# Developer-Zer0/GIF-synthesis-with-Discrete-Diffusion

Hardware: NVIDIA B200
Metric: reverse_step_token_updates_per_sec (higher is better)
Workload: dtype f32

## Files before the change

### gif-synthesis-with-discrete-diffusion_b200/csrc/d3pm_step_rows.cuh

```cuda
#pragma once

#include "d3pm_common.cuh"

namespace d3pm {

struct StepParams {
  const float* logits_c;
  const float* logits_u;
  const int64_t* x_t;
  const int64_t* t;
  const float* coef_table;
  const float* gumbel;
  int64_t* x_prev;
  float* post;
  float* recon;
  float* gap;
  uint32_t* status;
  int32_t B, N, K, T;
  int64_t pitch_logits, pitch_gumbel, pitch_out;
  float guidance_scale;
  int32_t sample_mode;
  int32_t gumbel_is_uniform;
  uint64_t seed, offset;
  int64_t row_offset;
  float thin_factor;
  int64_t rows;
  int32_t sample_from;
  float* score;
  const float* sharpen;
  float* winner_post;
  int32_t logits_dtype;
  PhiloxRoundKeys keys;
};

__device__ __forceinline__ float to_log2_units(float m) { return __fmul_rn(m, kLog2e); }

__device__ __forceinline__ float ln_rel_sum(float M, float S) {
  const float m2 = to_log2_units(M);
  const float delta = -fmaf(M, kLog2e, -m2);
  return kLn2 * (lg2(S) + delta);
}

struct RowMath {
  float A, Bc;
  float Pj;
  float PK;
  float Ptot;
  uint32_t j;

  __device__ __forceinline__ void init(const RowCoef& cf, bool masked, float pj, uint32_t jj, int K) {
    init(cf, masked, pj, 1.0f - pj, jj, K);
  }
  __device__ __forceinline__ void init(const RowCoef& cf, bool masked, float pj, float qj, uint32_t jj, int K) {
    j = jj;
    const float eL = masked ? cf.W + kTiny : fmaf(cf.W, qj, fmaf(cf.WS, pj, kTiny));
    A = cf.A;
    Bc = cf.BO * eL;
    Pj = masked ? 0.0f : fmaf(pj, cf.AS, cf.BOS * eL);
    PK = fmaf(cf.PK1, eL, cf.PK0);
    Ptot = masked ? fmaf(static_cast<float>(K), Bc, A) + PK
                  : fmaf(static_cast<float>(K - 1), Bc, A * qj) + Pj + PK;
  }
  __device__ __forceinline__ void init_recon(float pj, uint32_t jj) {
    j = jj;
    A = 1.0f, Bc = 0.0f, Pj = pj, PK = kPFloor, Ptot = 1.0f + kPFloor;
  }
  __device__ __forceinline__ float post_of(uint32_t k, float e, float r) const {
    const float p = fminf(fmaxf(e * r, kPFloor), 1.0f);
    const float P = (k == j) ? Pj : fmaf(p, A, Bc);
    return log_prob_clamped(P);
  }
  __device__ __forceinline__ float post_self() const { return log_prob_clamped(Pj); }
  __device__ __forceinline__ float post_mask() const { return log_prob_clamped(PK); }
};

constexpr float kDefaultThin = 8.0f;
struct ThinRule {
  float scaleA, thrB, accept;
  __device__ __forceinline__ ThinRule(const RowMath& rm, float thin_factor) {
    const float c = thin_factor > 0.f ? thin_factor : kDefaultThin;
    const float inv = __fdividef(c, rm.Ptot);
    scaleA = rm.A * inv * 0.0078125f;
    thrB = fmaf(rm.Bc * inv, 0.0078125f, 1.0f) + 2.384185791015625e-7f;
    accept = -lg2(inv) * kLn2 + 0.02f;
  }
};

constexpr int kRowThreads = 256;

template <int NV, int NW, typename Sync>
__device__ __forceinline__ void group_max_sum_n(float (&m)[NV], float (&s)[NV], float* scratch, Sync sync) {
  const int lane = threadIdx.x & 31, warp = (threadIdx.x >> 5) % NW;
#pragma unroll
  for (int v = 0; v < NV; ++v) {
    const float mw = warp_max(m[v]);
    const float sw =
        warp_sum(m[v] == -CUDART_INF_F ? 0.0f : s[v] * ex2(to_log2_units(m[v]) - to_log2_units(mw)));
    if (lane == 0) {
      scratch[(2 * v) * NW + warp] = mw;
      scratch[(2 * v + 1) * NW + warp] = sw;
    }
  }
  sync();
#pragma unroll
  for (int v = 0; v < NV; ++v) {
    float M = scratch[(2 * v) * NW];
#pragma unroll
    for (int w = 1; w < NW; ++w) M = fmaxf(M, scratch[(2 * v) * NW + w]);
    const float M2 = to_log2_units(M);
    float S = 0.0f;
#pragma unroll
    for (int w = 0; w < NW; ++w) {
      const float mwv = scratch[(2 * v) * NW + w];
      S += (mwv == -CUDART_INF_F) ? 0.0f : scratch[(2 * v + 1) * NW + w] * ex2(to_log2_units(mwv) - M2);
    }
    m[v] = M;
    s[v] = S;
  }
}

template <int V, bool HAS_U, bool THIN>
__global__ void __launch_bounds__(kRowThreads) step_rows_kernel(const StepParams p) {
  constexpr int NW = kRowThreads / 32;
  __shared__ float sred[3][4 * NW];
  __shared__ unsigned long long skey[2][NW];
  __shared__ float sgap[NW];
  const CtaSync sync;

  const int tid = threadIdx.x;
  const int64_t row = blockIdx.x;
  const int b = static_cast<int>(row / p.N);
  const int K = p.K, nq = K >> 2;

  long long tt = p.t[b];
  long long jj = p.x_t[row];
  uint32_t st = 0;
  if (tt < 0 || tt >= p.T) {
    st |= D3PM_STATUS_BAD_T;
    tt = tt < 0 ? 0 : p.T - 1;
  }
  if (jj < 0 || jj > K) {
    st |= D3PM_STATUS_BAD_TOKEN;
    jj = K;
  }
  if (st != 0 && tid == 0 && p.status != nullptr) atomicOr(p.status, st);
  const bool masked = (jj == K);
  const uint32_t j = static_cast<uint32_t>(jj);
  const RowCoef cf = load_row_coef(p.coef_table, static_cast<int>(tt), masked);

  const float* __restrict__ rc = p.logits_c + row * p.pitch_logits;
  const float* __restrict__ ru = HAS_U ? p.logits_u + row * p.pitch_logits : nullptr;

  float x[V][4], z[V][4];
  int nvalid = 0;
#pragma unroll
  for (int i = 0; i < V; ++i) {
    const int q = tid + i * kRowThreads;
    if (q < nq) {
      nvalid = i + 1;
      const float4 a = ld_stream4(rc + 4 * q);
      x[i][0] = a.x, x[i][1] = a.y, x[i][2] = a.z, x[i][3] = a.w;
      if (HAS_U) {
        const float4 c = ld_stream4(ru + 4 * q);
        z[i][0] = c.x, z[i][1] = c.y, z[i][2] = c.z, z[i][3] = c.w;
      }
    } else {
#pragma unroll
      for (int e = 0; e < 4; ++e) x[i][e] = -CUDART_INF_F, z[i][e] = -CUDART_INF_F;
    }
  }
  float xj = 0.f, zj = 0.f;
  if (!masked) {
    xj = __ldg(rc + j);
    if (HAS_U) zj = __ldg(ru + j);
  }

  float m[2] = {-CUDART_INF_F, -CUDART_INF_F}, s[2] = {0.f, 0.f};
#pragma unroll
  for (int i = 0; i < V; ++i)
#pragma unroll
    for (int e = 0; e < 4; ++e) {
      m[0] = fmaxf(m[0], x[i][e]);
      if (HAS_U) m[1] = fmaxf(m[1], z[i][e]);
    }
  {
// ... 260 lines not shown
```

### gif-synthesis-with-discrete-diffusion_b200/csrc/d3pm_step_stream.cuh

```cuda
#pragma once

#include <cuda_fp16.h>

#include <type_traits>

#include "d3pm_step_rows.cuh"

namespace d3pm {

constexpr int kGroupThreads = 128;
constexpr int kGroupWarps = kGroupThreads / 32;
constexpr int kGroupsPerCta = 4;
constexpr int kStreamThreads = kGroupThreads * kGroupsPerCta;
constexpr int kCandPerRow = 30;
constexpr float kStreamThin = 8.0f;
constexpr float kRedoThin = 16.0f;
constexpr int kCoefSmemRows = 256;
struct RowInfo {
  float A, Bc, Pj, PK, accept;
  uint32_t j;
  int32_t rel;
  int32_t pad;
};

template <int NP, int CPT, bool HAS_U>
struct StreamShape {
  static_assert(CPT == 8 || (CPT == 16 && !HAS_U), "64 classes per thread only fit in registers without the second tensor");
  static constexpr int K = 1024 * NP;
  static constexpr int GT = 256 * NP / CPT;
  static constexpr int NW = GT / 32;
  static constexpr int NG = kStreamThreads / GT;
  static constexpr int SB = 128 / NG;
  static constexpr int RC = 8192 / NG;
  static constexpr int PS = 128 / GT;
  static constexpr int NCALL = CPT / 2;
  static_assert(GT >= 32 && GT <= 128 && NG <= 16, "unsupported group shape");
};

template <int NP, int CPT, bool HAS_U>
struct __align__(128) GroupSmem {
  using Sh = StreamShape<NP, CPT, HAS_U>;
  float c[1024 * NP];
  float u[HAS_U ? 1024 * NP : 4];
  alignas(16) float red[3][6 * 4];
  unsigned long long full;
  unsigned long long keys[4];
  uint32_t redo_cnt;
  uint32_t pad;
  RowInfo info[Sh::SB];
  uint32_t cand_cnt[Sh::SB];
  uint32_t cand_k[Sh::SB][kCandPerRow];
  float cand_p[Sh::SB][kCandPerRow];
  int32_t redo[Sh::RC];
};

__device__ __forceinline__ uint32_t smem_u32(const void* p) {
  return static_cast<uint32_t>(__cvta_generic_to_shared(p));
}
__device__ __forceinline__ void mbar_init(unsigned long long* bar, uint32_t count) {
  asm volatile("mbarrier.init.shared::cta.b64 [%0], %1;" ::"r"(smem_u32(bar)), "r"(count) : "memory");
  asm volatile("fence.mbarrier_init.release.cluster;" ::: "memory");
}
__device__ __forceinline__ void mbar_expect_tx(unsigned long long* bar, uint32_t bytes) {
  asm volatile("mbarrier.arrive.expect_tx.shared::cta.b64 _, [%0], %1;" ::"r"(smem_u32(bar)), "r"(bytes) : "memory");
}
__device__ __forceinline__ void mbar_wait(unsigned long long* bar, uint32_t parity) {
  const uint32_t addr = smem_u32(bar);
  uint32_t done;
  do {
    asm volatile(
        "{\n\t.reg .pred p;\n\t"
        "mbarrier.try_wait.parity.shared::cta.b64 p, [%1], %2;\n\t"
        "selp.u32 %0, 1, 0, p;\n\t}"
        : "=r"(done)
        : "r"(addr), "r"(parity)
        : "memory");
  } while (!done);
}
__device__ __forceinline__ void tma_load_row(void* dst, const void* src, uint32_t bytes, unsigned long long* bar) {
  asm volatile(
      "cp.async.bulk.shared::cluster.global.mbarrier::complete_tx::bytes [%0], [%1], %2, [%3];"
      ::"r"(smem_u32(dst)), "l"(src), "r"(bytes), "r"(smem_u32(bar))
      : "memory");
}
__device__ __forceinline__ void group_bar(int id) {
  asm volatile("bar.sync %0, %1;" ::"r"(id), "n"(kGroupThreads) : "memory");
}
struct GroupSync {
  int id;
  __device__ __forceinline__ void operator()() const { group_bar(id); }
};
template <int NW>
struct StreamSync {
  int id;
  __device__ __forceinline__ void operator()() const {
    if (NW == 1) __syncwarp();
    else asm volatile("bar.sync %0, %1;" ::"r"(id), "n"(32 * NW) : "memory");
  }
};
__device__ __forceinline__ float4 lds4(const float* p) { return *reinterpret_cast<const float4*>(p); }
template <int LD>
struct LogitType {
  static constexpr uint32_t kBytes = LD == D3PM_LOGITS_F32 ? 4u : 2u;
  static __device__ __forceinline__ float2 widen(uint32_t pair) {
    if constexpr (LD == D3PM_LOGITS_BF16) {
      return make_float2(__uint_as_float(pair << 16), __uint_as_float(pair & 0xffff0000u));
    } else {
      return __half22float2(*reinterpret_cast<const __half2*>(&pair));
    }
  }
  static __device__ __forceinline__ void chunk(const float* stage, int q, float2& lo, float2& hi) {
    if constexpr (LD == D3PM_LOGITS_F32) {
      const float4 a = lds4(stage + 4 * q);
      lo = make_float2(a.x, a.y), hi = make_float2(a.z, a.w);
    } else {
      const uint2 raw = *reinterpret_cast<const uint2*>(reinterpret_cast<const unsigned char*>(stage) + 8 * q);
      lo = widen(raw.x), hi = widen(raw.y);
    }
  }
  static __device__ __forceinline__ float one(const float* stage, uint32_t k) {
    if constexpr (LD == D3PM_LOGITS_F32) {
      return stage[k];
    } else {
      const uint32_t h = reinterpret_cast<const unsigned short*>(stage)[k];
      if constexpr (LD == D3PM_LOGITS_BF16) return __uint_as_float(h << 16);
      else return __half2float(__ushort_as_half(static_cast<unsigned short>(h)));
    }
  }
  static __device__ __forceinline__ const void* row(const float* base, unsigned long long elements) {
    return reinterpret_cast<const unsigned char*>(base) + elements * kBytes;
  }
};
template <int NW>
__device__ __forceinline__ float4 lds_warps(const float* p, float neutral) {
  if (NW == 4) return lds4(p);
  const float2 a = *reinterpret_cast<const float2*>(p);
  return make_float4(a.x, a.y, neutral, neutral);
}
template <int NW, int NV, typename Sync>
__device__ __forceinline__ void stream_max_sum(float (&m)[NV], float (&s)[NV], float* scratch, Sync sync) {
  const int lane = threadIdx.x & 31, warp = (threadIdx.x >> 5) & (NW - 1);
#pragma unroll
  for (int v = 0; v < NV; ++v) {
    const float mw = warp_max(m[v]);
    const float mw2 = to_log2_units(mw);
    const float sw = warp_sum(s[v] * ex2(to_log2_units(m[v]) - mw2));
    if (NW == 1) {
      m[v] = mw, s[v] = sw;
    } else if (lane == 0) {
      scratch[(3 * v) * 4 + warp] = mw;
      scratch[(3 * v + 1) * 4 + warp] = mw2;
      scratch[(3 * v + 2) * 4 + warp] = sw;
    }
  }
  sync();
  if constexpr (NW > 1) {
#pragma unroll
  for (int v = 0; v < NV; ++v) {
    const float4 mw = lds_warps<NW>(scratch + (3 * v) * 4, -CUDART_INF_F), mw2 = lds_warps<NW>(scratch + (3 * v + 1) * 4, 0.f);
    const float4 sw = lds_warps<NW>(scratch + (3 * v + 2) * 4, 0.f);
    if (NW == 4) {
      const float M = fmaxf(fmaxf(mw.x, mw.y), fmaxf(mw.z, mw.w));
      const float M2 = to_log2_units(M);
      m[v] = M;
      s[v] = fmaf(sw.x, ex2(mw2.x - M2), fmaf(sw.y, ex2(mw2.y - M2), fmaf(sw.z, ex2(mw2.z - M2), sw.w * ex2(mw2.w - M2))));
    } else {
      const float M = fmaxf(mw.x, mw.y);
      const float M2 = to_log2_units(M);
      m[v] = M;
      s[v] = fmaf(sw.x, ex2(mw2.x - M2), sw.y * ex2(mw2.y - M2));
    }
  }
  }
}

__device__ __forceinline__ float warp_min(float x) {
  float m;
  asm volatile("redux.sync.min.f32 %0, %1, 0xffffffff;" : "=f"(m) : "f"(x));
  return m;
}

template <int NW, int NV, typename Sync>
__device__ __forceinline__ void stream_max(float* mx, float* scratch, Sync sync) {
  const int lane = threadIdx.x & 31, warp = (threadIdx.x >> 5) & (NW - 1);
#pragma unroll
  for (int v = 0; v < NV; ++v) {
    const float a = warp_max(mx[v]);
    if (NW == 1) mx[v] = a;
    else if (lane == 0) scratch[v * 4 + warp] = a;
  }
  sync();
  if constexpr (NW > 1) {
#pragma unroll
  for (int v = 0; v < NV; ++v) {
    const float4 a = lds_warps<NW>(scratch + v * 4, -CUDART_INF_F);
    mx[v] = fmaxf(fmaxf(a.x, a.y), fmaxf(a.z, a.w));
  }
  }
}

template <int NW, int NV, typename Sync>
__device__ __forceinline__ void stream_sum(float (&s)[NV], float* scratch, Sync sync) {
  const int lane = threadIdx.x & 31, warp = (threadIdx.x >> 5) & (NW - 1);
#pragma unroll
  for (int v = 0; v < NV; ++v) {
    const float sw = warp_sum(s[v]);
    if (NW == 1) s[v] = sw;
    else if (lane == 0) scratch[v * 4 + warp] = sw;
  }
  sync();
  if constexpr (NW > 1) {
#pragma unroll
  for (int v = 0; v < NV; ++v) {
    const float4 a = lds_warps<NW>(scratch + v * 4, 0.f);
    s[v] = (a.x + a.y) + (a.z + a.w);
  }
  }
}

template <int NW, typename Sync>
__device__ __forceinline__ unsigned long long stream_max_u64(unsigned long long key, unsigned long long* scratch, Sync sync) {
  const int lane = threadIdx.x & 31, warp = (threadIdx.x >> 5) & (NW - 1);
  key = warp_max_u64(key);
  if (NW == 1) {
    sync();
    return key;
  }
  if (lane == 0) scratch[warp] = key;
  sync();
  unsigned long long best = scratch[0];
#pragma unroll
  for (int w = 1; w < NW; ++w) best = scratch[w] > best ? scratch[w] : best;
  return best;
}

template <int NP, int CPT, bool HAS_U>
__device__ __noinline__ void score_batch(GroupSmem<NP, CPT, HAS_U>& S, int nslots, const ParamNoiseStream& rng, const StepParams& p, int G,
                                         int first_row) {
  using Sh = StreamShape<NP, CPT, HAS_U>;
  constexpr uint32_t K = 1024u * NP;
  const int lane = threadIdx.x & 31, warp = (threadIdx.x >> 5) & (Sh::NW - 1);
  const int sub = lane & 15;
  for (int slot = 2 * warp + (lane >> 4); slot - (lane >> 4) < nslots; slot += 2 * Sh::NW) {
    unsigned long long key = 0ull;
    float lp = 0.f;
    const bool live = slot < nslots;
    RowInfo ri;
    ri.accept = 0.f, ri.rel = 0;
    uint32_t cnt = 0;
    if (live) {
      ri = S.info[slot];
      cnt = S.cand_cnt[slot];
      const uint32_t n = cnt < static_cast<uint32_t>(kCandPerRow) ? cnt : static_cast<uint32_t>(kCandPerRow);
      const uint64_t grow = static_cast<uint64_t>(p.row_offset + (first_row + ri.rel * G));
      for (uint32_t item = static_cast<uint32_t>(sub); item < n + 2u; item += 16u) {
        uint32_t k = 0;
        float P = 0.f;
        bool have = false;
        if (item < n) {
          k = S.cand_k[slot][item];
          const float pe = fminf(fmaxf(S.cand_p[slot][item], kPFloor), 1.0f);
          P = fmaf(pe, ri.A, ri.Bc);
          have = (k != ri.j);
        } else if (item == n) {
          k = K, P = ri.PK, have = true;
        } else if (ri.j != K) {
          k = ri.j, P = ri.Pj, have = true;
        }
        if (have) {
          const float lpk = log_prob_clamped(P);
          const float sc = lpk + gumbel_from_uniform(uniform_from_draw(rng.draw(k, grow)));
          const unsigned long long kk = pack_key(sc, k);
          if (kk > key) key = kk, lp = lpk;
        }
      }
    }
    const unsigned long long mine = key;
#pragma unroll
    for (int o = 8; o > 0; o >>= 1) {
      const unsigned long long other = __shfl_xor_sync(0xffffffffu, key, o);
      key = other > key ? other : key;
    }
    const bool accepted = live && cnt <= static_cast<uint32_t>(kCandPerRow) && key_score(key) >= ri.accept;
    if (live && sub == 0) {
      if (accepted) {
        p.x_prev[first_row + ri.rel * G] = key_class(key);
      } else {
        S.redo[atomicAdd(&S.redo_cnt, 1u)] = ri.rel;
      }
      S.cand_cnt[slot] = 0;
    }
    if (p.winner_post != nullptr && accepted && mine == key && mine != 0ull) p.winner_post[first_row + ri.rel * G] = lp;
  }
}

template <int NP, int CPT, bool HAS_U, bool RECON, int LD = D3PM_LOGITS_F32>
__global__ void __launch_bounds__(kStreamThreads, 1) step_stream_kernel(const __grid_constant__ StepParams p) {
  extern __shared__ __align__(128) unsigned char smem_raw[];
  using Sh = StreamShape<NP, CPT, HAS_U>;
  using Smem = GroupSmem<NP, CPT, HAS_U>;
  constexpr int K = Sh::K, GT = Sh::GT, NW = Sh::NW, NG = Sh::NG, PS = Sh::PS, NCALL = Sh::NCALL;
  constexpr int NC = CPT;
  using LT = LogitType<LD>;
  constexpr uint32_t kRowBytes = K * LT::kBytes;
  uint32_t tid;
  asm volatile("mov.u32 %0, %%tid.x;" : "=r"(tid));
  const int g = tid / GT;
  const int tg = tid % GT;
  Smem& S = reinterpret_cast<Smem*>(smem_raw)[g];
  const StreamSync<NW> sync{g + 1};
  const int G = static_cast<int>(gridDim.x) * NG;
  const int first_row = g * static_cast<int>(gridDim.x) + static_cast<int>(blockIdx.x);
  const int rows = static_cast<int>(p.rows);
  const uint32_t pitch = static_cast<uint32_t>(p.pitch_logits);
  const bool exact_mode = (p.sample_mode == D3PM_SAMPLE_PHILOX_EXACT);
  if (tg == 0) {
    mbar_init(&S.full, 1);
    S.redo_cnt = 0;
    if (!exact_mode && first_row < rows) {
      const unsigned long long at = static_cast<unsigned long long>(static_cast<uint32_t>(first_row)) * pitch;
      mbar_expect_tx(&S.full, HAS_U ? 2 * kRowBytes : kRowBytes);
      tma_load_row(S.c, LT::row(p.logits_c, at), kRowBytes, &S.full);
      if (HAS_U) tma_load_row(S.u, LT::row(p.logits_u, at), kRowBytes, &S.full);
    }
  }
  float* coef_s = reinterpret_cast<float*>(smem_raw + sizeof(Smem) * NG);
  const bool coef_in_smem = p.T <= kCoefSmemRows;
  if (coef_in_smem) {
    for (int i = tid; i < p.T * 16; i += kStreamThreads)
      coef_s[i] = __ldg(p.coef_table + static_cast<size_t>(i >> 4) * D3PM_COEF_STRIDE + (i & 15));
  }
  const ParamNoiseStream rng(NoiseKeysParam(p.keys), p.offset);
  const float thin_c = p.thin_factor > 0.f ? p.thin_factor : kStreamThin;
  for (int i = tg; i < Sh::SB; i += GT) S.cand_cnt[i] = 0;
  __syncthreads();

  auto issue_row = [&](int row) {
    const unsigned long long at = static_cast<unsigned long long>(static_cast<uint32_t>(row)) * pitch;
    asm volatile("fence.proxy.async.shared::cta;" ::: "memory");
    mbar_expect_tx(&S.full, HAS_U ? 2 * kRowBytes : kRowBytes);
    tma_load_row(S.c, LT::row(p.logits_c, at), kRowBytes, &S.full);
    if (HAS_U) tma_load_row(S.u, LT::row(p.logits_u, at), kRowBytes, &S.full);
  };
  auto slot_lo = [](int c) { return (c / PS) * 2 * PS + (c % PS); };

  uint32_t phase = 0;
  uint32_t status_bits = 0;
#ifdef D3PM_STREAM_TIMING
  auto now_ns = [] { unsigned long long v; asm volatile("mov.u64 %0, %%globaltimer;" : "=l"(v)); return v; };
  const unsigned long long tm_start = now_ns();
  unsigned long long tm_main = 0;
  uint32_t tm_rows = 0, tm_redo = 0;
#endif

  auto process_row = [&](auto exact_c, int row, int next_row, uint32_t j, int tt, int slot, int rel) {
    constexpr bool exact = decltype(exact_c)::value;
    const bool masked = (j == static_cast<uint32_t>(K));
    mbar_wait(&S.full, phase);
    phase ^= 1u;

    float2 x[NC][2], z[HAS_U ? NC : 1][2];
#pragma unroll
    for (int i = 0; i < NC; ++i) {
      const int q = GT * i + tg;
      LT::chunk(S.c, q, x[i][0], x[i][1]);
      if (HAS_U) LT::chunk(S.u, q, z[i][0], z[i][1]);
    }
    auto e_of = [&](int i, int h) -> float2& {
      if constexpr (HAS_U) return z[i][h];
      else return x[i][h];
    };
    const float xj = masked ? 0.f : LT::one(S.c, j);
    const float zj = (HAS_U && !masked) ? LT::one(S.u, j) : 0.f;

    float am[2] = {0.f, 0.f};
    if (HAS_U) {
      am[0] = fmaxf(fmaxf(fabsf(x[0][0].x), fabsf(x[0][0].y)), fmaxf(fabsf(x[0][1].x), fabsf(x[0][1].y)));
      am[1] = fmaxf(fmaxf(fabsf(z[0][0].x), fabsf(z[0][0].y)), fmaxf(fabsf(z[0][1].x), fabsf(z[0][1].y)));
    }
#pragma unroll
    for (int i = 1; i < NC; ++i) {
      if (HAS_U)
        am[0] = fmaxf(fmaxf(am[0], fabsf(x[i][0].x)), fmaxf(fabsf(x[i][0].y), fmaxf(fabsf(x[i][1].x), fabsf(x[i][1].y))));
      if (HAS_U)
        am[1] = fmaxf(fmaxf(am[1], fabsf(z[i][0].x)), fmaxf(fabsf(z[i][0].y), fmaxf(fabsf(z[i][1].x), fabsf(z[i][1].y))));
    }
    if (HAS_U) stream_max<NW, 2>(am, S.red[0], sync);
    else sync();
    if (!exact && tg == 0 && next_row >= 0) issue_row(next_row);

    const uint64_t grow = static_cast<uint64_t>(p.row_offset + row);

    float My2, rSy, r, yj;
    const float2 l2e = make_float2(kLog2e, kLog2e);
    if (HAS_U) {
      const float gs = p.guidance_scale, og = 1.0f - gs;
      const float2 gs2 = make_float2(gs, gs), og2 = make_float2(og, og);
      float my = -CUDART_INF_F;
      constexpr float kLnK = NP == 4 ? 8.3178f : (NP == 2 ? 7.6247f : 6.9315f);
      constexpr float kSafeAbs = 0.5f * (69.99f - kLnK);
      const bool no_clamp = (am[0] <= kSafeAbs) && (am[1] <= kSafeAbs) && (fabsf(gs) * am[0] + fabsf(og) * am[1] <= 160.0f);
      if (no_clamp) {
#pragma unroll
        for (int i = 0; i < NC; ++i)
#pragma unroll
          for (int h = 0; h < 2; ++h) {
            const float2 y = __ffma2_rn(gs2, x[i][h], __fmul2_rn(og2, z[i][h]));
            x[i][h] = y;
            my = fmaxf(my, fmaxf(y.x, y.y));
          }
        yj = fmaf(gs, xj, og * zj);
      } else {
        float mx[2], s[2];
        mx[0] = fmaxf(fmaxf(x[0][0].x, x[0][0].y), fmaxf(x[0][1].x, x[0][1].y));
        mx[1] = fmaxf(fmaxf(z[0][0].x, z[0][0].y), fmaxf(z[0][1].x, z[0][1].y));
#pragma unroll
        for (int i = 1; i < NC; ++i) {
          mx[0] = fmaxf(fmaxf(mx[0], x[i][0].x), fmaxf(x[i][0].y, fmaxf(x[i][1].x, x[i][1].y)));
          mx[1] = fmaxf(fmaxf(mx[1], z[i][0].x), fmaxf(z[i][0].y, fmaxf(z[i][1].x, z[i][1].y)));
        }
        stream_max<NW, 2>(mx, S.red[2], sync);
        mx[0] = fmaxf(mx[0], -3.0e38f), mx[1] = fmaxf(mx[1], -3.0e38f);
        {
          const float mc2 = to_log2_units(mx[0]), mu2 = to_log2_units(mx[1]);
          const float2 nmc = make_float2(-mc2, -mc2), nmu = make_float2(-mu2, -mu2);
          float2 sc[2] = {make_float2(0.f, 0.f), make_float2(0.f, 0.f)}, su[2] = {sc[0], sc[0]};
#pragma unroll
          for (int i = 0; i < NC; ++i)
#pragma unroll
            for (int h = 0; h < 2; ++h) {
              const float2 ac = __ffma2_rn(x[i][h], l2e, nmc), au = __ffma2_rn(z[i][h], l2e, nmu);
              sc[h] = __fadd2_rn(sc[h], make_float2(ex2(ac.x), ex2(ac.y)));
              su[h] = __fadd2_rn(su[h], make_float2(ex2(au.x), ex2(au.y)));
            }
          s[0] = (sc[0].x + sc[0].y) + (sc[1].x + sc[1].y);
          s[1] = (su[0].x + su[0].y) + (su[1].x + su[1].y);
        }
        stream_sum<NW, 2>(s, S.red[2] + 2 * 4, sync);
        const float lnSc = ln_rel_sum(mx[0], s[0]), lnSu = ln_rel_sum(mx[1], s[1]);
        const float ta = kClampLo + lnSc, tb = kClampLo + lnSu;
        const float C = fmaf(-gs, lnSc, -og * lnSu);
        const float2 nMc = make_float2(-mx[0], -mx[0]), nMu = make_float2(-mx[1], -mx[1]), C2 = make_float2(C, C);
#pragma unroll
        for (int i = 0; i < NC; ++i)
#pragma unroll
          for (int h = 0; h < 2; ++h) {
            float2 a = __fadd2_rn(x[i][h], nMc), b = __fadd2_rn(z[i][h], nMu);
            a.x = fmaxf(a.x, ta), a.y = fmaxf(a.y, ta);
            b.x = fmaxf(b.x, tb), b.y = fmaxf(b.y, tb);
            const float2 y = __ffma2_rn(gs2, a, __ffma2_rn(og2, b, C2));
            x[i][h] = y;
            my = fmaxf(my, fmaxf(y.x, y.y));
          }
        yj = fmaf(gs, fmaxf(xj - mx[0], ta), fmaf(og, fmaxf(zj - mx[1], tb), C));
      }
      const float my2 = to_log2_units(my);
      {
        const float2 nmy = make_float2(-my2, -my2);
        float2 sy[2] = {make_float2(0.f, 0.f), make_float2(0.f, 0.f)};
#pragma unroll
        for (int i = 0; i < NC; ++i)
#pragma unroll
          for (int h = 0; h < 2; ++h) {
            const float2 ay = __ffma2_rn(x[i][h], l2e, nmy);
            const float2 ey = make_float2(ex2(ay.x), ex2(ay.y));
            e_of(i, h) = ey;
            sy[h] = __fadd2_rn(sy[h], ey);
          }
        float mm[1] = {my}, ss[1] = {(sy[0].x + sy[0].y) + (sy[1].x + sy[1].y)};
        stream_max_sum<NW, 1>(mm, ss, S.red[1], sync);
        My2 = to_log2_units(mm[0]);
        rSy = __fdividef(1.0f, ss[0]);
      }
      r = ex2(my2 - My2) * rSy;
    } else {
      float mx[1];
      mx[0] = fmaxf(fmaxf(x[0][0].x, x[0][0].y), fmaxf(x[0][1].x, x[0][1].y));
#pragma unroll
      for (int i = 1; i < NC; ++i) mx[0] = fmaxf(fmaxf(mx[0], x[i][0].x), fmaxf(x[i][0].y, fmaxf(x[i][1].x, x[i][1].y)));
      mx[0] = fmaxf(mx[0], -3.0e38f);
      const float mc2 = to_log2_units(mx[0]);
      const float2 nmc = make_float2(-mc2, -mc2);
      float2 sc[2] = {make_float2(0.f, 0.f), make_float2(0.f, 0.f)};
#pragma unroll
      for (int i = 0; i < NC; ++i)
#pragma unroll
        for (int h = 0; h < 2; ++h) {
          const float2 ac = __ffma2_rn(x[i][h], l2e, nmc);
          const float2 ec = make_float2(ex2(ac.x), ex2(ac.y));
          e_of(i, h) = ec;
          sc[h] = __fadd2_rn(sc[h], ec);
        }
      float ss[1] = {(sc[0].x + sc[0].y) + (sc[1].x + sc[1].y)};
      stream_max_sum<NW, 1>(mx, ss, S.red[1], sync);
      My2 = to_log2_units(mx[0]);
      rSy = __fdividef(1.0f, ss[0]);
      r = ex2(mc2 - My2) * rSy;
      yj = xj;
    }
    const float pj = masked ? 0.f : fminf(fmaxf(ex2(fmaf(yj, kLog2e, -My2)) * rSy, kPFloor), 1.0f);
    RowCoef cf;
    if (coef_in_smem) {
      const float* crow = coef_s + tt * 16 + (masked ? 0 : 8);
      cf = row_coef_from(lds4(crow), lds4(crow + 4), masked);
    } else {
      cf = load_row_coef(p.coef_table, tt, masked);
    }
    RowMath rm;
    if (RECON) {
      rm.init_recon(masked ? 0.f : pj, masked ? static_cast<uint32_t>(K) + 1u : j);
      if (tg == 0 && p.score != nullptr) p.score[row] = fminf(fmaxf(rSy, kPFloor), 1.0f);
    } else {
      rm.init(cf, masked, pj, j, K);
    }

    if constexpr (!exact) {
      const ThinRule thin(rm, thin_c);
      const float thrA = r * thin.scaleA, nthrB = -thin.thrB;
      const float2 tA2 = make_float2(thrA, thrA);
      if (tg == 0) {
        RowInfo ri;
        ri.A = rm.A, ri.Bc = rm.Bc, ri.Pj = rm.Pj, ri.PK = rm.PK, ri.accept = thin.accept;
        ri.j = j, ri.rel = rel, ri.pad = 0;
        S.info[slot] = ri;
      }
#pragma unroll
      for (int c0 = 0; c0 < NCALL; c0 += 4) {
        uint4 cws[4];
#pragma unroll
        for (int c = 0; c < 4; ++c) cws[c] = rng.coarse(ParamNoiseStream::coarse_call_of_chunk(GT * slot_lo(c0 + c) + tg), grow);
#pragma unroll
        for (int c = 0; c < 4; ++c) {
          const int lo = slot_lo(c0 + c);
          const uint32_t w4[4] = {cws[c].x, cws[c].y, cws[c].z, cws[c].w};
          float slack = -4.0f;
#pragma unroll
          for (int w = 0; w < 4; ++w) {
            const float2 nf = make_float2(__uint_as_float(__byte_perm(w4[w], 0xbf80u, 0x5410)),
                                          __uint_as_float(__byte_perm(w4[w], 0xbf80u, 0x5432)));
            const float2 d = __ffma2_rn(e_of(lo + (w >> 1) * PS, w & 1), tA2, nf);
            slack = fmaxf(slack, fmaxf(d.x, d.y));
          }
          if (slack >= nthrB) {
#pragma unroll
            for (int w = 0; w < 4; ++w)
#pragma unroll
              for (int hl = 0; hl < 2; ++hl) {
                const float2 ee = e_of(lo + (w >> 1) * PS, w & 1);
                const float e = hl ? ee.y : ee.x;
                const uint32_t h16 = hl ? (w4[w] >> 16) : (w4[w] & 0xffffu);
                const float nf = __uint_as_float(0xbf800000u | h16);
                if (fmaf(e, thrA, nf) >= nthrB) {
                  const uint32_t pos = atomicAdd(&S.cand_cnt[slot], 1u);
                  if (pos < static_cast<uint32_t>(kCandPerRow)) {
                    S.cand_k[slot][pos] = 4u * (GT * (lo + (w >> 1) * PS) + tg) + 2u * (w & 1) + hl;
                    S.cand_p[slot][pos] = e * r;
                  }
                }
              }
          }
        }
      }
      return;
    } else {
    unsigned long long best = 0ull;
    float best_lp = 0.f;
    bool settled = false;
    if (!exact_mode) {
      const ThinRule thin2(rm, (p.thin_factor > 0.f && p.thin_factor < 0.01f) ? p.thin_factor : kRedoThin);
      const float thrA = r * thin2.scaleA;
      const float2 tA2 = make_float2(thrA, thrA), tB2 = make_float2(thin2.thrB, thin2.thrB);
#pragma unroll
      for (int c = 0; c < NCALL; ++c) {
        const int lo = slot_lo(c);
        const uint4 cw = rng.coarse(ParamNoiseStream::coarse_call_of_chunk(GT * lo + tg), grow);
        const uint32_t w4[4] = {cw.x, cw.y, cw.z, cw.w};
        uint32_t hits = 0;
        float ev[8];
#pragma unroll
        for (int w = 0; w < 4; ++w) {
          const float2 ee = e_of(lo + (w >> 1) * PS, w & 1);
          ev[2 * w] = ee.x, ev[2 * w + 1] = ee.y;
          const float2 nf = make_float2(__uint_as_float(__byte_perm(w4[w], 0xbf80u, 0x5410)),
                                        __uint_as_float(__byte_perm(w4[w], 0xbf80u, 0x5432)));
          const float2 d = __ffma2_rn(ee, tA2, __fadd2_rn(tB2, nf));
          hits |= (d.x >= 0.0f ? 1u : 0u) << (2 * w);
          hits |= (d.y >= 0.0f ? 1u : 0u) << (2 * w + 1);
        }
        while (hits != 0) {
          const int b = __ffs(hits) - 1;
          hits &= hits - 1;
          float e = 0.f;
#pragma unroll
          for (int q = 0; q < 8; ++q) e = (b == q) ? ev[q] : e;
          const uint32_t k = 4u * (GT * (lo + (b >> 2) * PS) + tg) + static_cast<uint32_t>(b & 3);
          if (k != j) {
            const float lpk = rm.post_of(k, e, r);
            const unsigned long long key = pack_key(lpk + gumbel_from_uniform(uniform_from_draw(rng.draw(k, grow))), k);
            if (key > best) best = key, best_lp = lpk;
          }
        }
      }
      if (tg == 0) {
        const float lpk = rm.post_mask();
        const unsigned long long key = pack_key(lpk + gumbel_from_uniform(uniform_from_draw(rng.draw(K, grow))), K);
        if (key > best) best = key, best_lp = lpk;
      }
      if (tg == GT - 1 && !masked) {
        const float lpk = rm.post_self();
        const unsigned long long key = pack_key(lpk + gumbel_from_uniform(uniform_from_draw(rng.draw(j, grow))), j);
        if (key > best) best = key, best_lp = lpk;
      }
      const unsigned long long mine = best;
      best = stream_max_u64<NW>(best, S.keys, sync);
      settled = key_score(best) >= thin2.accept;
      if (settled) {
        if (p.winner_post != nullptr && mine == best) p.winner_post[row] = best_lp;
      } else {
        best = 0ull;
        sync();
      }
    }
    if (!settled) {
#pragma unroll
      for (int i = 0; i < NC; ++i) {
        const float2 a = e_of(i, 0), b = e_of(i, 1);
        *reinterpret_cast<float4*>(S.c + 4 * (GT * i + tg)) = make_float4(a.x, a.y, b.x, b.y);
      }
#pragma unroll 1
      for (int i = 0; i < NC; ++i) {
        const uint32_t q = static_cast<uint32_t>(GT) * i + tg;
        const float4 e4 = lds4(S.c + 4 * q);
        const float ev[4] = {e4.x, e4.y, e4.z, e4.w};
        const uint4 cw = rng.coarse(ParamNoiseStream::coarse_call_of_chunk(q), grow);
        const uint4 fw = rng.fine(q >> 2, grow);
#pragma unroll
        for (int e = 0; e < 4; ++e) {
          const uint32_t k = 4u * q + e;
          const uint32_t mdraw =
              (ParamNoiseStream::half_of(cw, (((q >> 7) & 1u) << 2) | e) << 7) | ParamNoiseStream::low7_of(fw, ((q & 3u) << 2) | e);
          const float lpk = rm.post_of(k, ev[e], r);
          const unsigned long long key = pack_key(lpk + gumbel_from_uniform(uniform_from_draw(mdraw)), k);
          if (key > best) best = key, best_lp = lpk;
        }
      }
      if (tg == 0) {
        const float lpk = rm.post_mask();
        const unsigned long long key = pack_key(lpk + gumbel_from_uniform(uniform_from_draw(rng.draw(K, grow))), K);
        if (key > best) best = key, best_lp = lpk;
      }
      const unsigned long long mine = best;
      best = stream_max_u64<NW>(best, S.keys, sync);
      if (p.winner_post != nullptr && mine == best) p.winner_post[row] = best_lp;
    }
    if (tg == 0) {
      p.x_prev[row] = key_class(best);
      if (next_row >= 0) issue_row(next_row);
    }
    }
  };

  const int N = p.N;
  auto token_of = [&](int r_) { return static_cast<long long>(p.x_t[r_]); };
  auto time_of = [&](int b_) { return static_cast<long long>(p.t[b_]); };
  auto checked = [&](long long tt, long long jj, int& t_cur, uint32_t& j_cur) {
    if (static_cast<unsigned long long>(tt) >= static_cast<unsigned long long>(p.T)) {
      status_bits |= D3PM_STATUS_BAD_T;
      tt = tt < 0 ? 0 : p.T - 1;
    }
    if (static_cast<unsigned long long>(jj) > static_cast<unsigned long long>(K)) {
      status_bits |= D3PM_STATUS_BAD_TOKEN;
      jj = K;
    }
    t_cur = static_cast<int>(tt), j_cur = static_cast<uint32_t>(jj);
    asm volatile("" : "+r"(t_cur), "+r"(j_cur) : : "memory");
  };
  if (!exact_mode) {
    const int stepB = G / N, stepR = G % N;
    int vb = first_row / N, vr = first_row % N;
    int row = first_row < rows ? first_row : -1;
    long long jj = 0, tt = 0;
    if (row >= 0) {
      jj = token_of(row);
      tt = time_of(vb);
    }
    int it = 0, in_batch = 0;
    while (row >= 0) {
      int t_cur;
      uint32_t j_cur;
      checked(tt, jj, t_cur, j_cur);
      const int next = row + G < rows ? row + G : -1;
      vb += stepB, vr += stepR;
      if (vr >= N) vr -= N, ++vb;
      if (next >= 0) {
        jj = token_of(next);
        tt = time_of(vb);
      }
      process_row(std::false_type{}, row, next, j_cur, t_cur, in_batch, it);
#ifdef D3PM_STREAM_TIMING
      ++tm_rows;
#endif
      row = next;
      ++it;
      if (++in_batch == Sh::SB || row < 0) {
        sync();
        score_batch<NP, CPT, HAS_U>(S, in_batch, rng, p, G, first_row);
        sync();
        in_batch = 0;
      }
    }
  }
#ifdef D3PM_STREAM_TIMING
  tm_main = now_ns();
#endif
  {
    const uint32_t n2 = exact_mode ? (first_row < rows ? static_cast<uint32_t>((rows - first_row + G - 1) / G) : 0u) : S.redo_cnt;
    auto row_at = [&](uint32_t i) { return first_row + (exact_mode ? static_cast<int>(i) : S.redo[i]) * G; };
    if (n2 > 0) {
      if (!exact_mode) status_bits |= D3PM_STATUS_FALLBACK;
      int row = row_at(0);
      if (tg == 0) issue_row(row);
      long long jj = token_of(row), tt = time_of(row / N);
      for (uint32_t i = 0; i < n2; ++i) {
        int t_cur;
        uint32_t j_cur;
        checked(tt, jj, t_cur, j_cur);
        const int next = (i + 1 < n2) ? row_at(i + 1) : -1;
        if (next >= 0) {
          jj = token_of(next);
          tt = time_of(next / N);
        }
        process_row(std::true_type{}, row, next, j_cur, t_cur, 0, 0);
#ifdef D3PM_STREAM_TIMING
        ++tm_redo;
#endif
        row = next;
      }
    }
  }
#ifdef D3PM_STREAM_TIMING
  if (tg == 0 && p.status != nullptr) {
    const unsigned long long tm_end = now_ns();
    uint32_t* o = p.status + 8 * (blockIdx.x * NG + g);
    uint32_t smid;
    asm volatile("mov.u32 %0, %%smid;" : "=r"(smid));
    o[0] = static_cast<uint32_t>(tm_start), o[1] = static_cast<uint32_t>(tm_start >> 32);
    o[2] = static_cast<uint32_t>(tm_main - tm_start), o[3] = static_cast<uint32_t>(tm_end - tm_start);
    o[4] = tm_rows, o[5] = tm_redo, o[6] = smid, o[7] = 0;
  }
#else
  if (status_bits != 0 && tg == 0 && p.status != nullptr) atomicOr(p.status, status_bits);
#endif
}

constexpr long long kStreamMinRows = 1024;

inline bool stream_kernel_supports(const StepParams& p) {
  if (p.sample_mode != D3PM_SAMPLE_PHILOX && p.sample_mode != D3PM_SAMPLE_PHILOX_EXACT) return false;
  if (p.post != nullptr || p.recon != nullptr || p.gap != nullptr || p.x_prev == nullptr) return false;
  if (p.sharpen != nullptr || (p.score != nullptr && p.sample_from != D3PM_FROM_RECON)) return false;
  if (p.K != 1024 && p.K != 2048 && p.K != 4096) return false;
  if (p.pitch_logits >= (1LL << 32)) return false;
  if (p.logits_dtype != D3PM_LOGITS_F32 && (p.sample_from == D3PM_FROM_RECON || p.pitch_logits % 8 != 0)) return false;
  return true;
}

inline long long stream_kernel_max_rows() {
  int dev = 0, sms = 0;
  if (cudaGetDevice(&dev) != cudaSuccess) return 0;
  if (cudaDeviceGetAttribute(&sms, cudaDevAttrMultiProcessorCount, dev) != cudaSuccess) return 0;
  return 8192LL * sms;
}

template <int NP, int CPT, bool HAS_U, bool RECON, int LD>
int launch_step_stream_r(const StepParams& p, cudaStream_t s) {
  using Sh = StreamShape<NP, CPT, HAS_U>;
  int dev = 0, sms = 0;
  if (cudaGetDevice(&dev) != cudaSuccess) return D3PM_ERR_CUDA;
  if (cudaDeviceGetAttribute(&sms, cudaDevAttrMultiProcessorCount, dev) != cudaSuccess) return D3PM_ERR_CUDA;
  const size_t smem = sizeof(GroupSmem<NP, CPT, HAS_U>) * Sh::NG + kCoefSmemRows * 16 * sizeof(float);
  auto kern = step_stream_kernel<NP, CPT, HAS_U, RECON, LD>;
  if (cudaFuncSetAttribute(kern, cudaFuncAttributeMaxDynamicSharedMemorySize, static_cast<int>(smem)) != cudaSuccess)
    return D3PM_ERR_CUDA;
  kern<<<static_cast<unsigned>(sms), kStreamThreads, smem, s>>>(p);
  return D3PM_OK;
}

template <int NP, int CPT, bool HAS_U>
int launch_step_stream_t(const StepParams& p, cudaStream_t s) {
  if (p.logits_dtype == D3PM_LOGITS_F16)
    return p.sample_from == D3PM_FROM_RECON ? D3PM_ERR_UNSUPPORTED : launch_step_stream_r<NP, CPT, HAS_U, false, D3PM_LOGITS_F16>(p, s);
  if (p.logits_dtype == D3PM_LOGITS_BF16)
    return p.sample_from == D3PM_FROM_RECON ? D3PM_ERR_UNSUPPORTED : launch_step_stream_r<NP, CPT, HAS_U, false, D3PM_LOGITS_BF16>(p, s);
  return p.sample_from == D3PM_FROM_RECON ? launch_step_stream_r<NP, CPT, HAS_U, true, D3PM_LOGITS_F32>(p, s)
                                          : launch_step_stream_r<NP, CPT, HAS_U, false, D3PM_LOGITS_F32>(p, s);
}

inline int launch_step_stream(const StepParams& p, cudaStream_t s) {
  const bool has_u = p.logits_u != nullptr;
  switch (p.K) {
    case 1024: return has_u ? launch_step_stream_t<1, 8, true>(p, s) : launch_step_stream_t<1, 8, false>(p, s);
    case 2048: return has_u ? launch_step_stream_t<2, 8, true>(p, s) : launch_step_stream_t<2, 16, false>(p, s);
    case 4096: return has_u ? launch_step_stream_t<4, 8, true>(p, s) : launch_step_stream_t<4, 16, false>(p, s);
    default: return D3PM_ERR_UNSUPPORTED;
  }
}

}
```

Baseline: 206.7 million.

## Add atomic ticket pool for tail rows and enable programmatic dependent launch

The last rounds of rows, a fixed count per group, move from a static row-to-group stride to a dynamic pool. Groups claim rows from a per-stream global atomic ticket counter, which the last finishing group resets, and the pool uses its own thinning factor. The kernel now launches with programmatic stream serialization and griddepcontrol wait/launch_dependents, so its prologue can overlap the previous kernel. The host also caches the SM count and the shared-memory attribute to cut per-launch API overhead. The cost is extra global atomics, per-row syncs in the pool loop, and host-side slot bookkeeping for the ticket counters.

```diff
diff --git a/gif-synthesis-with-discrete-diffusion_b200/csrc/d3pm_step_rows.cuh b/gif-synthesis-with-discrete-diffusion_b200/csrc/d3pm_step_rows.cuh
--- a/gif-synthesis-with-discrete-diffusion_b200/csrc/d3pm_step_rows.cuh
+++ b/gif-synthesis-with-discrete-diffusion_b200/csrc/d3pm_step_rows.cuh
@@ -31,6 +31,7 @@
   float* winner_post;
   int32_t logits_dtype;
   PhiloxRoundKeys keys;
+  unsigned long long* tickets = nullptr;
 };
 
 __device__ __forceinline__ float to_log2_units(float m) { return __fmul_rn(m, kLog2e); }
diff --git a/gif-synthesis-with-discrete-diffusion_b200/csrc/d3pm_step_stream.cuh b/gif-synthesis-with-discrete-diffusion_b200/csrc/d3pm_step_stream.cuh
--- a/gif-synthesis-with-discrete-diffusion_b200/csrc/d3pm_step_stream.cuh
+++ b/gif-synthesis-with-discrete-diffusion_b200/csrc/d3pm_step_stream.cuh
@@ -2,6 +2,11 @@
 
 #include <cuda_fp16.h>
 
+#include <atomic>
+#include <map>
+#include <mutex>
+#include <thread>
+#include <tuple>
 #include <type_traits>
 
 #include "d3pm_step_rows.cuh"
@@ -15,11 +20,13 @@
 constexpr int kCandPerRow = 30;
 constexpr float kStreamThin = 8.0f;
 constexpr float kRedoThin = 16.0f;
+constexpr int kStreamPoolRounds = 12;
+constexpr float kPoolThin = 12.0f;
 constexpr int kCoefSmemRows = 256;
 struct RowInfo {
   float A, Bc, Pj, PK, accept;
   uint32_t j;
-  int32_t rel;
+  int32_t row;
   int32_t pad;
 };
 
@@ -46,7 +53,7 @@
   unsigned long long full;
   unsigned long long keys[4];
   uint32_t redo_cnt;
-  uint32_t pad;
+  int32_t ticket[2];
   RowInfo info[Sh::SB];
   uint32_t cand_cnt[Sh::SB];
   uint32_t cand_k[Sh::SB][kCandPerRow];
@@ -235,8 +242,7 @@
 }
 
 template <int NP, int CPT, bool HAS_U>
-__device__ __noinline__ void score_batch(GroupSmem<NP, CPT, HAS_U>& S, int nslots, const ParamNoiseStream& rng, const StepParams& p, int G,
-                                         int first_row) {
+__device__ __noinline__ void score_batch(GroupSmem<NP, CPT, HAS_U>& S, int nslots, const ParamNoiseStream& rng, const StepParams& p) {
   using Sh = StreamShape<NP, CPT, HAS_U>;
   constexpr uint32_t K = 1024u * NP;
   const int lane = threadIdx.x & 31, warp = (threadIdx.x >> 5) & (Sh::NW - 1);
@@ -246,13 +252,13 @@
     float lp = 0.f;
     const bool live = slot < nslots;
     RowInfo ri;
-    ri.accept = 0.f, ri.rel = 0;
+    ri.accept = 0.f, ri.row = 0;
     uint32_t cnt = 0;
     if (live) {
       ri = S.info[slot];
       cnt = S.cand_cnt[slot];
       const uint32_t n = cnt < static_cast<uint32_t>(kCandPerRow) ? cnt : static_cast<uint32_t>(kCandPerRow);
-      const uint64_t grow = static_cast<uint64_t>(p.row_offset + (first_row + ri.rel * G));
+      const uint64_t grow = static_cast<uint64_t>(p.row_offset + ri.row);
       for (uint32_t item = static_cast<uint32_t>(sub); item < n + 2u; item += 16u) {
         uint32_t k = 0;
         float P = 0.f;
@@ -284,13 +290,13 @@
     const bool accepted = live && cnt <= static_cast<uint32_t>(kCandPerRow) && key_score(key) >= ri.accept;
     if (live && sub == 0) {
       if (accepted) {
-        p.x_prev[first_row + ri.rel * G] = key_class(key);
+        p.x_prev[ri.row] = key_class(key);
       } else {
-        S.redo[atomicAdd(&S.redo_cnt, 1u)] = ri.rel;
+        S.redo[atomicAdd(&S.redo_cnt, 1u)] = ri.row;
       }
       S.cand_cnt[slot] = 0;
     }
-    if (p.winner_post != nullptr && accepted && mine == key && mine != 0ull) p.winner_post[first_row + ri.rel * G] = lp;
+    if (p.winner_post != nullptr && accepted && mine == key && mine != 0ull) p.winner_post[ri.row] = lp;
   }
 }
 
@@ -314,15 +320,21 @@
   const int rows = static_cast<int>(p.rows);
   const uint32_t pitch = static_cast<uint32_t>(p.pitch_logits);
   const bool exact_mode = (p.sample_mode == D3PM_SAMPLE_PHILOX_EXACT);
+  constexpr bool kPool = LD == D3PM_LOGITS_F32;
+  const int n_static = (kPool && p.tickets != nullptr && !exact_mode) ? max(rows - kStreamPoolRounds * G, 0) : rows;
   if (tg == 0) {
     mbar_init(&S.full, 1);
     S.redo_cnt = 0;
-    if (!exact_mode && first_row < rows) {
-      const unsigned long long at = static_cast<unsigned long long>(static_cast<uint32_t>(first_row)) * pitch;
-      mbar_expect_tx(&S.full, HAS_U ? 2 * kRowBytes : kRowBytes);
-      tma_load_row(S.c, LT::row(p.logits_c, at), kRowBytes, &S.full);
-      if (HAS_U) tma_load_row(S.u, LT::row(p.logits_u, at), kRowBytes, &S.full);
-    }
+  }
+  const ParamNoiseStream rng(NoiseKeysParam(p.keys), p.offset);
+  float thin_c = p.thin_factor > 0.f ? p.thin_factor : kStreamThin;
+  for (int i = tg; i < Sh::SB; i += GT) S.cand_cnt[i] = 0;
+  asm volatile("griddepcontrol.wait;" ::: "memory");
+  if (tg == 0 && !exact_mode && first_row < n_static) {
+    const unsigned long long at = static_cast<unsigned long long>(static_cast<uint32_t>(first_row)) * pitch;
+    mbar_expect_tx(&S.full, HAS_U ? 2 * kRowBytes : kRowBytes);
+    tma_load_row(S.c, LT::row(p.logits_c, at), kRowBytes, &S.full);
+    if (HAS_U) tma_load_row(S.u, LT::row(p.logits_u, at), kRowBytes, &S.full);
   }
   float* coef_s = reinterpret_cast<float*>(smem_raw + sizeof(Smem) * NG);
   const bool coef_in_smem = p.T <= kCoefSmemRows;
@@ -330,9 +342,6 @@
     for (int i = tid; i < p.T * 16; i += kStreamThreads)
       coef_s[i] = __ldg(p.coef_table + static_cast<size_t>(i >> 4) * D3PM_COEF_STRIDE + (i & 15));
   }
-  const ParamNoiseStream rng(NoiseKeysParam(p.keys), p.offset);
-  const float thin_c = p.thin_factor > 0.f ? p.thin_factor : kStreamThin;
-  for (int i = tg; i < Sh::SB; i += GT) S.cand_cnt[i] = 0;
   __syncthreads();
 
   auto issue_row = [&](int row) {
@@ -349,15 +358,18 @@
 #ifdef D3PM_STREAM_TIMING
   auto now_ns = [] { unsigned long long v; asm volatile("mov.u64 %0, %%globaltimer;" : "=l"(v)); return v; };
   const unsigned long long tm_start = now_ns();
-  unsigned long long tm_main = 0;
+  unsigned long long tm_main = 0, tm_first = 0;
   uint32_t tm_rows = 0, tm_redo = 0;
 #endif
 
-  auto process_row = [&](auto exact_c, int row, int next_row, uint32_t j, int tt, int slot, int rel) {
+  auto process_row = [&](auto exact_c, int row, int next_row, uint32_t j, int tt, int slot) {
     constexpr bool exact = decltype(exact_c)::value;
     const bool masked = (j == static_cast<uint32_t>(K));
     mbar_wait(&S.full, phase);
     phase ^= 1u;
+#ifdef D3PM_STREAM_TIMING
+    if (tm_first == 0) tm_first = now_ns();
+#endif
 
     float2 x[NC][2], z[HAS_U ? NC : 1][2];
 #pragma unroll
@@ -521,7 +533,7 @@
       if (tg == 0) {
         RowInfo ri;
         ri.A = rm.A, ri.Bc = rm.Bc, ri.Pj = rm.Pj, ri.PK = rm.PK, ri.accept = thin.accept;
-        ri.j = j, ri.rel = rel, ri.pad = 0;
+        ri.j = j, ri.row = row, ri.pad = 0;
         S.info[slot] = ri;
       }
 #pragma unroll
@@ -675,53 +687,54 @@
     t_cur = static_cast<int>(tt), j_cur = static_cast<uint32_t>(jj);
     asm volatile("" : "+r"(t_cur), "+r"(j_cur) : : "memory");
   };
+  uint32_t redone = 0;
+  int taken = 0, in_batch = 0;
   if (!exact_mode) {
     const int stepB = G / N, stepR = G % N;
     int vb = first_row / N, vr = first_row % N;
-    int row = first_row < rows ? first_row : -1;
+    int row = first_row < n_static ? first_row : -1;
     long long jj = 0, tt = 0;
     if (row >= 0) {
       jj = token_of(row);
       tt = time_of(vb);
     }
-    int it = 0, in_batch = 0;
     while (row >= 0) {
       int t_cur;
       uint32_t j_cur;
       checked(tt, jj, t_cur, j_cur);
-      const int next = row + G < rows ? row + G : -1;
+      const int next = row + G < n_static ? row + G : -1;
       vb += stepB, vr += stepR;
       if (vr >= N) vr -= N, ++vb;
       if (next >= 0) {
         jj = token_of(next);
         tt = time_of(vb);
       }
-      process_row(std::false_type{}, row, next, j_cur, t_cur, in_batch, it);
+      process_row(std::false_type{}, row, next, j_cur, t_cur, in_batch);
 #ifdef D3PM_STREAM_TIMING
       ++tm_rows;
 #endif
       row = next;
-      ++it;
+      ++taken;
       if (++in_batch == Sh::SB || row < 0) {
         sync();
-        score_batch<NP, CPT, HAS_U>(S, in_batch, rng, p, G, first_row);
+        score_batch<NP, CPT, HAS_U>(S, in_batch, rng, p);
         sync();
         in_batch = 0;
       }
     }
   }
+  for (bool pool = n_static < rows;; pool = false) {
 #ifdef D3PM_STREAM_TIMING
-  tm_main = now_ns();
+    tm_main = now_ns();
 #endif
-  {
     const uint32_t n2 = exact_mode ? (first_row < rows ? static_cast<uint32_t>((rows - first_row + G - 1) / G) : 0u) : S.redo_cnt;
-    auto row_at = [&](uint32_t i) { return first_row + (exact_mode ? static_cast<int>(i) : S.redo[i]) * G; };
-    if (n2 > 0) {
+    auto row_at = [&](uint32_t i) { return exact_mode ? first_row + static_cast<int>(i) * G : S.redo[i]; };
+    if (n2 > redone) {
       if (!exact_mode) status_bits |= D3PM_STATUS_FALLBACK;
-      int row = row_at(0);
+      int row = row_at(redone);
       if (tg == 0) issue_row(row);
       long long jj = token_of(row), tt = time_of(row / N);
-      for (uint32_t i = 0; i < n2; ++i) {
+      for (uint32_t i = redone; i < n2; ++i) {
         int t_cur;
         uint32_t j_cur;
         checked(tt, jj, t_cur, j_cur);
@@ -730,14 +743,69 @@
           jj = token_of(next);
           tt = time_of(next / N);
         }
-        process_row(std::true_type{}, row, next, j_cur, t_cur, 0, 0);
+        process_row(std::true_type{}, row, next, j_cur, t_cur, 0);
 #ifdef D3PM_STREAM_TIMING
         ++tm_redo;
 #endif
         row = next;
       }
-    }
-  }
+      redone = n2;
+    }
+    if (!pool) break;
+    {
+      const int pool_rows = rows - n_static;
+      auto take = [&]() -> int {
+        if (taken < Sh::RC) {
+          const int tk = static_cast<int>(static_cast<uint32_t>(atomicAdd(p.tickets, 1ull)));
+          if (tk < pool_rows) {
+            ++taken;
+            return n_static + tk;
+          }
+        }
+        if ((atomicAdd(p.tickets, 1ull << 32) >> 32) == static_cast<unsigned long long>(G - 1)) atomicExch(p.tickets, 0ull);
+        return -1;
+      };
+      if (!(p.thin_factor > 0.f)) thin_c = kPoolThin;
+      int row = -1, next = -1;
+      long long jj = 0, tt = 0;
+      if (tg == 0) {
+        row = take();
+        next = row >= 0 ? take() : -1;
+        if (row >= 0) issue_row(row);
+        S.ticket[0] = row, S.ticket[1] = next;
+      }
+      sync();
+      row = S.ticket[0], next = S.ticket[1];
+      if (row >= 0) {
+        jj = token_of(row);
+        tt = time_of(row / N);
+      }
+      while (row >= 0) {
+        int t_cur;
+        uint32_t j_cur;
+        checked(tt, jj, t_cur, j_cur);
+        if (next >= 0) {
+          jj = token_of(next);
+          tt = time_of(next / N);
+        }
+        const int after = (tg == 0 && next >= 0) ? take() : -1;
+        process_row(std::false_type{}, row, next, j_cur, t_cur, in_batch);
+#ifdef D3PM_STREAM_TIMING
+        ++tm_rows;
+#endif
+        if (tg == 0) S.ticket[1] = after;
+        sync();
+        row = next, next = S.ticket[1];
+        if (++in_batch == Sh::SB || row < 0) {
+          sync();
+          score_batch<NP, CPT, HAS_U>(S, in_batch, rng, p);
+          sync();
+          in_batch = 0;
+        }
+      }
+    }
+  }
+  asm volatile("griddepcontrol.launch_dependents;" ::: "memory");
 #ifdef D3PM_STREAM_TIMING
   if (tg == 0 && p.status != nullptr) {
     const unsigned long long tm_end = now_ns();
@@ -746,7 +814,7 @@
     asm volatile("mov.u32 %0, %%smid;" : "=r"(smid));
     o[0] = static_cast<uint32_t>(tm_start), o[1] = static_cast<uint32_t>(tm_start >> 32);
     o[2] = static_cast<uint32_t>(tm_main - tm_start), o[3] = static_cast<uint32_t>(tm_end - tm_start);
-    o[4] = tm_rows, o[5] = tm_redo, o[6] = smid, o[7] = 0;
+    o[4] = tm_rows, o[5] = tm_redo, o[6] = smid, o[7] = tm_first != 0 ? static_cast<uint32_t>(tm_first - tm_start) : 0u;
   }
 #else
   if (status_bits != 0 && tg == 0 && p.status != nullptr) atomicOr(p.status, status_bits);
@@ -765,24 +833,85 @@
   return true;
 }
 
+constexpr int kStreamMaxDevices = 64;
+inline int stream_sm_count(int dev) {
+  static std::atomic<int> cached[kStreamMaxDevices];
+  if (dev < 0 || dev >= kStreamMaxDevices) return 0;
+  int sms = cached[dev].load(std::memory_order_relaxed);
+  if (sms == 0) {
+    if (cudaDeviceGetAttribute(&sms, cudaDevAttrMultiProcessorCount, dev) != cudaSuccess) return 0;
+    cached[dev].store(sms, std::memory_order_relaxed);
+  }
+  return sms;
+}
+
 inline long long stream_kernel_max_rows() {
-  int dev = 0, sms = 0;
+  int dev = 0;
   if (cudaGetDevice(&dev) != cudaSuccess) return 0;
-  if (cudaDeviceGetAttribute(&sms, cudaDevAttrMultiProcessorCount, dev) != cudaSuccess) return 0;
-  return 8192LL * sms;
+  return 8192LL * stream_sm_count(dev);
+}
+
+constexpr int kStreamPoolSlots = 4096;
+__device__ unsigned long long g_stream_pool[kStreamPoolSlots];
+
+inline unsigned long long* stream_pool_slot(int dev, cudaStream_t s) {
+  static std::mutex mu;
+  static std::map<std::tuple<int, cudaStream_t, std::thread::id>, int> eager;
+  static int used[kStreamMaxDevices];
+  static unsigned long long* base[kStreamMaxDevices];
+  cudaStreamCaptureStatus cap = cudaStreamCaptureStatusNone;
+  if (cudaStreamIsCapturing(s, &cap) != cudaSuccess) {
+    (void)cudaGetLastError();
+    return nullptr;
+  }
+  std::lock_guard<std::mutex> lock(mu);
+  if (base[dev] == nullptr) {
+    void* a = nullptr;
+    if (cudaGetSymbolAddress(&a, g_stream_pool) != cudaSuccess) {
+      (void)cudaGetLastError();
+      return nullptr;
+    }
+    base[dev] = static_cast<unsigned long long*>(a);
+  }
+  int slot = -1;
+  if (cap == cudaStreamCaptureStatusActive) {
+    if (used[dev] < kStreamPoolSlots) slot = used[dev]++;
+  } else {
+    const auto key = std::make_tuple(dev, s, s == cudaStreamPerThread ? std::this_thread::get_id() : std::thread::id());
+    const auto it = eager.find(key);
+    if (it != eager.end()) slot = it->second;
+    else if (used[dev] < kStreamPoolSlots) eager.emplace(key, slot = used[dev]++);
+  }
+  return slot < 0 ? nullptr : base[dev] + slot;
 }
 
 template <int NP, int CPT, bool HAS_U, bool RECON, int LD>
-int launch_step_stream_r(const StepParams& p, cudaStream_t s) {
+int launch_step_stream_r(const StepParams& p_in, cudaStream_t s) {
   using Sh = StreamShape<NP, CPT, HAS_U>;
-  int dev = 0, sms = 0;
+  int dev = 0;
   if (cudaGetDevice(&dev) != cudaSuccess) return D3PM_ERR_CUDA;
-  if (cudaDeviceGetAttribute(&sms, cudaDevAttrMultiProcessorCount, dev) != cudaSuccess) return D3PM_ERR_CUDA;
+  const int sms = stream_sm_count(dev);
+  if (sms == 0) return D3PM_ERR_CUDA;
+  StepParams p = p_in;
+  p.tickets = (p.sample_mode == D3PM_SAMPLE_PHILOX && LD == D3PM_LOGITS_F32) ? stream_pool_slot(dev, s) : nullptr;
   const size_t smem = sizeof(GroupSmem<NP, CPT, HAS_U>) * Sh::NG + kCoefSmemRows * 16 * sizeof(float);
   auto kern = step_stream_kernel<NP, CPT, HAS_U, RECON, LD>;
-  if (cudaFuncSetAttribute(kern, cudaFuncAttributeMaxDynamicSharedMemorySize, static_cast<int>(smem)) != cudaSuccess)
-    return D3PM_ERR_CUDA;
-  kern<<<static_cast<unsigned>(sms), kStreamThreads, smem, s>>>(p);
+  static std::atomic<bool> smem_set[kStreamMaxDevices];
+  if (!smem_set[dev].load(std::memory_order_relaxed)) {
+    if (cudaFuncSetAttribute(kern, cudaFuncAttributeMaxDynamicSharedMemorySize, static_cast<int>(smem)) != cudaSuccess)
+      return D3PM_ERR_CUDA;
+    smem_set[dev].store(true, std::memory_order_relaxed);
+  }
+  cudaLaunchConfig_t cfg = {};
+  cfg.gridDim = dim3(static_cast<unsigned>(sms));
+  cfg.blockDim = dim3(kStreamThreads);
+  cfg.dynamicSmemBytes = smem;
+  cfg.stream = s;
+  cudaLaunchAttribute attr[1];
+  attr[0].id = cudaLaunchAttributeProgrammaticStreamSerialization;
+  attr[0].val.programmaticStreamSerializationAllowed = 1;
+  cfg.attrs = attr, cfg.numAttrs = 1;
+  if (cudaLaunchKernelEx(&cfg, kern, p) != cudaSuccess) return D3PM_ERR_CUDA;
   return D3PM_OK;
 }
 
```

Measured after the change: 208.4 million (median of 6 runs). Within noise of the previous version (+0.8%).
